# kaushik87599/Melo-GAN

Measured on AMD Instinct MI355X. Metric: piano-roll samples/sec (G+D step), batch=64 128x256 roll, higher is better.
Workload: dtype f32; 1 GPU; cfg2: 128x256 piano-roll, batch=64 per GPU, full G+D+emotion-D step (1 critic update incl. gradient penalty + 1 generator update); global_batch=64, T=256, C=128, parallelism=dp1, graph=True

## Files before the change

### include/melo_gan_hip.h

```cpp
#ifndef MELO_GAN_HIP_H
#define MELO_GAN_HIP_H

#include <stddef.h>
#include <stdint.h>

#ifdef __cplusplus
extern "C" {
#endif

typedef void* mg_stream_t;

enum { MG_ACT_NONE = 0, MG_ACT_RELU = 1, MG_ACT_LRELU = 2, MG_ACT_GELU = 3, MG_ACT_TANH = 4 };

typedef struct mg_epilogue {
    const float* bias;
    const float* scale;
    const float* shift;
    float* zout;
    int act;
    const float* gref;
    int gact;
    const float* emul;
    const float* gscale;
    int accumulate;
} mg_epilogue;

int mg_version(void);
const char* mg_last_error(void);

size_t mg_conv_workspace_bytes(int B, int Tout, int N);
int mg_conv1d_gather(const float* x, const float* w, float* y,
                     int B, int Tin, int Cin, int N, int K, int stride, int flip,
                     int w_sn, int w_sc, long xbs, long ybs,
                     const mg_epilogue* epi, void* work, size_t work_bytes, long lds_pad, mg_stream_t stream);

int mg_conv1d_scatter2(const float* x, const float* w, float* y,
                       int B, int Tin, int Cin, int N, int Tout,
                       int w_sn, int w_sc, long xbs, long ybs,
                       const mg_epilogue* epi, void* work, size_t work_bytes, mg_stream_t stream);

int mg_wq_relayout(const float* w, float* wq, int N, int Cc, int K, int w_sn, int w_sc, mg_stream_t stream);
int mg_conv16_supported(int B, int Tin, int Cin, int N, int transposed, int Tout);
int mg_conv16_plan(int B, int Tin, int N, int transposed, int* batch_rows_per_tile, int* part_rows, int* tile_rows);
int mg_conv16_poolable(int B, int Tin, int Cin, int N);
typedef struct mg_conv16_extra {
    float* part;
    float* pool;
    float pool_scale;
    int y_perm;
    const float* mix_real;
    const float* mix_alpha;
    float* mix_out;
    int mix_rows;
    const float* bnb_a;
    const float* bnb_z;
    const float* bnb_mean;
    const float* bnb_invstd;
    double* bnb_part;
    int bnb_act;
} mg_conv16_extra;
int mg_conv16(const float* x, const float* wq, float* y, int B, int Tin, int Cin, int N, int transposed, int Tout,
              long xbs, long ybs, const mg_epilogue* epi, const mg_conv16_extra* extra , mg_stream_t stream);
int mg_bn_train_bwd_parts(const double* part, int part_rows, const float* da, const float* a, const float* z, float* dz, long R,
                          int C, const float* gamma, const float* beta, const float* save_mean, const float* save_invstd,
                          float* dgamma, float* dbeta, int act, mg_stream_t stream);
int mg_bn_train_fwd_parts(const float* part, int part_rows_per_group, int groups, const float* z, float* a, long R, int C,
                          const float* gamma, const float* beta, float* running_mean, float* running_var, float momentum,
                          float eps, float* save_mean, float* save_invstd, int act, mg_stream_t stream);

#define MG_CHAIN_MAX_OPS 16
#define MG_CHAIN_SLOTS 6
#define MG_CHAIN_MAX_VEC 512
enum { MG_CH_LOAD = 1, MG_CH_STORE = 2, MG_CH_LAYERNORM = 3, MG_CH_LIN_FWD = 4, MG_CH_LIN_DGRAD = 5, MG_CH_SOFTMAX_CE = 6,
       MG_CH_DHEAD = 7, MG_CH_MEAN_T = 8, MG_CH_COPY = 9 };
typedef struct mg_chain_op {
    int kind;
    int a, b;
    int n0, n1;
    int act;
    int i0, i1;
    float f0;
    const float* p0; long ld0;
    const float* p1; long ld1;
    const float* p2; long ld2;
    const float* p3; long ld3;
    float* q0; long lq0;
    float* q1; long lq1;
    const int64_t* t0;
} mg_chain_op;
int mg_row_chain(const mg_chain_op* ops, int n_ops, int rows, mg_stream_t stream);
int mg_mean_scaled(const float* src, float* out, int n, float scale, mg_stream_t stream);
int mg_stamp(unsigned long long* dst, mg_stream_t stream);

size_t mg_linear_workspace_bytes(int M, int N, int K);
int mg_linear(const float* x, const float* w, float* y, int M, int K, int N, int w_sn, int w_sc,
              const mg_epilogue* epi, int perm_L, void* work, size_t work_bytes, mg_stream_t stream);
int mg_linear_route(int M, int K, int N, int w_sn, int w_sc, int perm_L, int x_aligned, int w_aligned,
                    int* kcontig, int* vec, int* ksplit);

int mg_conv1d_wino3_supported(int B, int T, int Cin, int N);
int mg_wino3_weights(const float* w, float* wt, int N, int Cin, long w_sn, long w_sc, int flip, mg_stream_t stream);
int mg_conv1d_wino3(const float* x, const float* wt, float* y, int B, int T, int Cin, int N, const mg_epilogue* epi,
                    long lds_pad, mg_stream_t stream);
#define MG_MAX_WINO_WJOBS 8
typedef struct mg_wino3_wjob {
    const float* w;
    float* wt;
    int N, Cin;
    long w_sn, w_sc;
    int flip;
} mg_wino3_wjob;
int mg_wino3_weights_multi(const mg_wino3_wjob* jobs, int n_jobs, mg_stream_t stream);

int mg_conv_tile_config(long m_rows, int N, int scatter2);
int mg_conv_plan(int B, int Tm, int Tout, int N, int Cin, int K, int stride, int scatter2, size_t work_bytes,
                 int* ksplit, int* cps);
int mg_conv_finish_vec(int N, long ybs, int tensors_aligned);

int mg_conv_thin_route(const float* x, long xbs, int Cin, int N, int K, int stride, int transposed);

typedef struct mg_epilogue_bf16 {
    const float* scale;
    const float* shift;
    void* zout;
    int act;
    const void* gref;
    int gact;
    const float* gscale;
    int accumulate;
} mg_epilogue_bf16;
int mg_wb_relayout(const float* w, void* wb, int N, int Cc, int K, int w_sn, int w_sc, int flip, mg_stream_t stream);
int mg_conv1d_s1_bf16_supported(int B, int T, int Cin, int N, int K);
int mg_conv1d_s1_bf16(const void* x, int x_f32, const void* wb, void* y, int y_f32, int B, int T, int Cin, int N, int K,
                      const mg_epilogue_bf16* epi, mg_stream_t stream);
int mg_meanT_fwd_bf16(const void* a, float* h, int B, int T, int C, mg_stream_t stream);
int mg_meanT_bwd_bf16(const float* dh, void* dz, const void* gref, int gact, const float* gscale, int B, int T, int C,
                      mg_stream_t stream);

size_t mg_wgrad_workspace_bytes(int A, int Bc, int K, int nb_total, int Ts);
int mg_wgrad(const float* s0, const float* l0, int nb0,
             const float* s1, const float* l1, int nb1,
             float* out, float* bias_out, int bias_from, int Ts, int Tl, int A, int Bc, int K, int stride,
             void* work, size_t work_bytes, mg_stream_t stream);

#define MG_MAX_WGRAD_JOBS 8
typedef struct mg_wgrad_job {
    const float* s0; const float* l0; int nb0;
    const float* s1; const float* l1; int nb1;
    float* out; float* bias_out; int bias_from;
    int Ts, Tl, A, Bc;
} mg_wgrad_job;
int mg_wgrad_multi(const mg_wgrad_job* jobs, int n_jobs, int K, int stride, void* work, size_t work_bytes,
                   mg_stream_t stream);

size_t mg_colsum_workspace_bytes(int C);
int mg_colsum(const float* x, long R, int C, float* sum, float* sumsq,
              void* work, size_t work_bytes, mg_stream_t stream);

size_t mg_bn_workspace_bytes(int C, int groups);
int mg_bn_train_fwd(const float* z, float* a, long R, int C, int groups, const float* gamma, const float* beta,
                    float* running_mean, float* running_var, float momentum, float eps,
                    float* save_mean, float* save_invstd, int act,
                    void* work, size_t work_bytes, mg_stream_t stream);
int mg_bn_train_bwd(const float* da, const float* a, const float* z, float* dz, long R, int C,
                    const float* gamma, const float* beta, const float* save_mean, const float* save_invstd,
                    float* dgamma, float* dbeta, int act,
                    void* work, size_t work_bytes, mg_stream_t stream);
int mg_bn_eval_fwd(const float* z, float* a, long R, int C, const float* gamma, const float* beta,
                   const float* running_mean, const float* running_var, float eps, int act,
                   mg_stream_t stream);
int mg_bn_fold(const float* gamma, const float* beta, const float* running_mean, const float* running_var,
               const float* conv_bias, float eps, float* scale, float* shift, int C, mg_stream_t stream);

int mg_meanT_fwd(const float* a, float* h, int B, int T, int C, mg_stream_t stream);
int mg_meanT_bwd(const float* dh, float* dz, int B, int T, int C, const float* gref, int gact, const float* gscale,
                 const float* mean_src, float* mean_out, int mean_n, float mean_scale, mg_stream_t stream);

int mg_layernorm_fwd(const float* x, float* y, float* xhat, int B, int D,
                     const float* gamma, const float* beta, float eps, mg_stream_t stream);
int mg_layernorm_bwd_params(const float* dy, const float* xhat, float* dgamma, float* dbeta,
                            int B, int D, mg_stream_t stream);

int mg_dhead_fwd(const float* f, const float* emb, const float* w, const float* bias, float* s,
                 int B, int Be, int F, int E, mg_stream_t stream);
int mg_dhead_bwd(const float* ds, const float* f, const float* w, float* dU, float* demb,
                 int B, int Be, int F, int E, int nb_emb, mg_stream_t stream);
// ... 238 lines not shown
```

### melo-gan_amd/_lib.py

```python
import ctypes as C
import os

_HERE = os.path.dirname(os.path.abspath(__file__))
LIB_PATH = os.path.join(_HERE, "libmelogan_hip.so")
if os.environ.get("MELO_LIB_VARIANT"):
    LIB_PATH = os.path.join(os.path.dirname(_HERE), "tools", "_build", "libmelogan_" + os.environ["MELO_LIB_VARIANT"] + ".so")

ACT_NONE, ACT_RELU, ACT_LRELU, ACT_GELU, ACT_TANH = 0, 1, 2, 3, 4

vp, i32, i64, f32, sz = C.c_void_p, C.c_int, C.c_long, C.c_float, C.c_size_t


class Epilogue(C.Structure):
    _fields_ = [("bias", vp), ("scale", vp), ("shift", vp), ("zout", vp), ("act", i32),
                ("gref", vp), ("gact", i32), ("emul", vp), ("gscale", vp), ("accumulate", i32)]


class EpilogueBf16(C.Structure):
    _fields_ = [("scale", vp), ("shift", vp), ("zout", vp), ("act", i32), ("gref", vp), ("gact", i32), ("gscale", vp),
                ("accumulate", i32)]


class Conv16Extra(C.Structure):
    _fields_ = [("part", vp), ("pool", vp), ("pool_scale", f32), ("y_perm", i32), ("mix_real", vp), ("mix_alpha", vp),
# ... 42 lines not shown


class WgradJob(C.Structure):
    _fields_ = [("s0", vp), ("l0", vp), ("nb0", i32), ("s1", vp), ("l1", vp), ("nb1", i32),
                ("out", vp), ("bias_out", vp), ("bias_from", i32), ("Ts", i32), ("Tl", i32), ("A", i32), ("Bc", i32)]


MAX_WGRAD_JOBS = 8


class WqEntry(C.Structure):
    _fields_ = [("start", i64), ("N", i32), ("Cc", i32), ("K", i32), ("w_sn", i32), ("w_sc", i32), ("dst", vp)]


MAX_WQ_ENTRIES = 8

MLP_MAX_HIDDEN, MLP_MAX_DIM, MLP_MAX_CLASSES = 4, 512, 32

VOICE_MAX_PARTIALS = 16


class Voice(C.Structure):
    _fields_ = [("n_partials", i32), ("mult", C.c_uint32 * VOICE_MAX_PARTIALS), ("weight", f32 * VOICE_MAX_PARTIALS),
                ("decay", f32 * VOICE_MAX_PARTIALS), ("attack", i32), ("release_tau", f32), ("release_len", i32), ("fs", f32)]


class MlpCls(C.Structure):
    _fields_ = [("n_hidden", i32), ("in_dim", i32), ("width", i32 * MLP_MAX_HIDDEN), ("n_classes", i32),
                ("w", vp * (MLP_MAX_HIDDEN + 1)), ("b", vp * (MLP_MAX_HIDDEN + 1)), ("z", vp * MLP_MAX_HIDDEN),
                ("a", vp * MLP_MAX_HIDDEN), ("dz", vp * MLP_MAX_HIDDEN), ("mask", vp * MLP_MAX_HIDDEN)]


SIGNATURES = {
    "mg_version": (i32, []),
    "mg_last_error": (C.c_char_p, []),
    "mg_conv_workspace_bytes": (sz, [i32, i32, i32]),
    "mg_conv1d_gather": (i32, [vp, vp, vp, i32, i32, i32, i32, i32, i32, i32, i32, i32, i64, i64, C.POINTER(Epilogue), vp, sz, i64, vp]),
    "mg_conv1d_scatter2": (i32, [vp, vp, vp, i32, i32, i32, i32, i32, i32, i32, i64, i64, C.POINTER(Epilogue), vp, sz, vp]),
    "mg_wq_relayout": (i32, [vp, vp, i32, i32, i32, i32, i32, vp]),
    "mg_conv16_supported": (i32, [i32, i32, i32, i32, i32, i32]),
    "mg_conv16_plan": (i32, [i32, i32, i32, i32, C.POINTER(i32), C.POINTER(i32), C.POINTER(i32)]),
    "mg_conv16": (i32, [vp, vp, vp, i32, i32, i32, i32, i32, i32, i64, i64, C.POINTER(Epilogue), C.POINTER(Conv16Extra), vp]),
    "mg_conv16_poolable": (i32, [i32, i32, i32, i32]),
    "mg_bn_train_fwd_parts": (i32, [vp, i32, i32, vp, vp, i64, i32, vp, vp, vp, vp, f32, f32, vp, vp, i32, vp]),
    "mg_linear_workspace_bytes": (sz, [i32, i32, i32]),
    "mg_linear": (i32, [vp, vp, vp, i32, i32, i32, i32, i32, C.POINTER(Epilogue), i32, vp, sz, vp]),
    "mg_conv_tile_config": (i32, [i64, i32, i32]),
    "mg_conv_plan": (i32, [i32, i32, i32, i32, i32, i32, i32, i32, sz, C.POINTER(i32), C.POINTER(i32)]),
    "mg_conv_finish_vec": (i32, [i32, i64, i32]),
    "mg_linear_route": (i32, [i32, i32, i32, i32, i32, i32, i32, i32, C.POINTER(i32), C.POINTER(i32), C.POINTER(i32)]),
    "mg_conv_thin_route": (i32, [vp, i64, i32, i32, i32, i32, i32]),
    "mg_wb_relayout": (i32, [vp, vp, i32, i32, i32, i32, i32, i32, vp]),
    "mg_conv1d_s1_bf16_supported": (i32, [i32, i32, i32, i32, i32]),
    "mg_conv1d_s1_bf16": (i32, [vp, i32, vp, vp, i32, i32, i32, i32, i32, i32, C.POINTER(EpilogueBf16), vp]),
    "mg_meanT_fwd_bf16": (i32, [vp, vp, i32, i32, i32, vp]),
    "mg_meanT_bwd_bf16": (i32, [vp, vp, vp, i32, vp, i32, i32, i32, vp]),
    "mg_wgrad_workspace_bytes": (sz, [i32, i32, i32, i32, i32]),
    "mg_wgrad": (i32, [vp, vp, i32, vp, vp, i32, vp, vp, i32, i32, i32, i32, i32, i32, i32, vp, sz, vp]),
    "mg_wgrad_multi": (i32, [vp, i32, i32, i32, vp, sz, vp]),
    "mg_colsum_workspace_bytes": (sz, [i32]),
    "mg_colsum": (i32, [vp, i64, i32, vp, vp, vp, sz, vp]),
    "mg_bn_workspace_bytes": (sz, [i32, i32]),
    "mg_bn_train_fwd": (i32, [vp, vp, i64, i32, i32, vp, vp, vp, vp, f32, f32, vp, vp, i32, vp, sz, vp]),
    "mg_bn_train_bwd": (i32, [vp, vp, vp, vp, i64, i32, vp, vp, vp, vp, vp, vp, i32, vp, sz, vp]),
    "mg_bn_train_bwd_parts": (i32, [vp, i32, vp, vp, vp, vp, i64, i32, vp, vp, vp, vp, vp, vp, i32, vp]),
    "mg_bn_eval_fwd": (i32, [vp, vp, i64, i32, vp, vp, vp, vp, f32, i32, vp]),
    "mg_bn_fold": (i32, [vp, vp, vp, vp, vp, f32, vp, vp, i32, vp]),
    "mg_meanT_fwd": (i32, [vp, vp, i32, i32, i32, vp]),
    "mg_layernorm_fwd": (i32, [vp, vp, vp, i32, i32, vp, vp, f32, vp]),
    "mg_layernorm_bwd_params": (i32, [vp, vp, vp, vp, i32, i32, vp]),
    "mg_dhead_fwd": (i32, [vp, vp, vp, vp, vp, i32, i32, i32, i32, vp]),
    "mg_dhead_bwd": (i32, [vp, vp, vp, vp, vp, i32, i32, i32, i32, i32, vp]),
    "mg_dhead_fwd_bwd": (i32, [vp, vp, vp, vp, vp, vp, vp, vp, i32, i32, i32, i32, i32, vp]),
    "mg_dhead_wgrad": (i32, [vp, vp, vp, vp, vp, vp, i32, i32, i32, i32, i32, vp, vp, f32, vp, vp, i32, vp]),
    "mg_meanT_bwd": (i32, [vp, vp, i32, i32, i32, vp, i32, vp, vp, vp, i32, f32, vp]),
    "mg_row_chain": (i32, [vp, i32, i32, vp]),
    "mg_mean_scaled": (i32, [vp, vp, i32, f32, vp]),
    "mg_stamp": (i32, [vp, vp]),
    "mg_spectral_norm_fwd": (i32, [vp, i32, i32, f32, vp]),
    "mg_spectral_norm_bwd": (i32, [vp, i32, vp]),
    "mg_conv1d_wino3_supported": (i32, [i32, i32, i32, i32]),
    "mg_wino3_weights": (i32, [vp, vp, i32, i32, i64, i64, i32, vp]),
    "mg_conv1d_wino3": (i32, [vp, vp, vp, i32, i32, i32, i32, vp, i64, vp]),
    "mg_wino3_weights_multi": (i32, [vp, i32, vp]),
    "mg_gp_interp": (i32, [vp, vp, vp, vp, i32, i64, vp]),
    "mg_gp_penalty": (i32, [vp, vp, vp, vp, f32, i32, i64, vp]),
    "mg_softmax_ce": (i32, [vp, vp, vp, vp, f32, i32, i32, vp]),
    "mg_axpby": (i32, [vp, vp, f32, f32, i64, vp]),
    "mg_copy_cols": (i32, [vp, i32, i32, vp, i32, i32, i32, i32, i32, vp]),
    "mg_transpose_bcl_blc": (i32, [vp, vp, i32, i32, i32, vp, i32, vp]),
    "mg_stage_rows": (i32, [vp, i32, i32, vp]),
    "mg_stage_rows_cursor": (i32, [vp, i32, i32, vp, i64, vp, vp, vp]),
    "mg_stage_augment": (i32, [vp, vp, i64, i32, i32, vp, vp, i32, vp, i64, vp, vp, vp, i32, C.POINTER(Augment), vp]),
    "mg_weighted_order": (i32, [vp, i64, vp, i64, C.c_uint64, C.c_uint64, vp]),
    "mg_ed_metrics_acc": (i32, [vp, vp, vp, i32, i32, vp, vp]),
    "mg_act_bwd": (i32, [vp, vp, i32, vp, vp, i64, vp]),
    "mg_rng_fill": (i32, [vp, i64, vp, i64, vp, i64, vp, i64, f32, C.c_uint64, vp, vp, vp, f32, f32, vp, i32, i32, vp, i64, vp, vp]),
    "mg_gen_inputs": (i32, [vp, vp, i32, vp, i32, vp, i32, vp, i32, f32, vp, i32, C.c_uint64, vp]),
    "mg_emotion_score": (i32, [vp, i32, i32, vp, vp, vp, vp, vp]),
    "mg_gen_inputs_mix": (i32, [vp, vp, vp, vp, i32, vp, i32, vp, i32, vp, i32, f32, vp, i32, C.c_uint64, vp]),
    "mg_path_d2": (i32, [vp, i32, i32, i32, vp, vp]),
    "mg_path_probs": (i32, [vp, vp, i32, i32, i32, i32, vp, vp, vp]),
    "mg_latent_rows": (i32, [vp, vp, i32, vp, i32, vp, vp, vp, vp, vp, vp, vp, vp, i32, i32, i32, C.c_uint64, vp, vp]),
    "mg_latent_cycle": (i32, [vp, vp, vp, i32, vp, i32, vp, vp, vp, i32, i32, vp, vp]),
    "mg_roll_encode": (i32, [vp, i64, vp, vp, i64, i32, i32, vp, vp, i64, vp, vp, vp]),
    "mg_window_votes": (i32, [vp, vp, i32, i32, i64, vp, vp, vp, vp, vp, vp]),
    "mg_ig_rows": (i32, [vp, vp, vp, vp, i32, i64, i32, i32, i32, i32, vp, vp, vp, vp]),
    "mg_ig_seed": (i32, [vp, vp, i64, i32, i32, i32, vp, vp, vp, vp, vp]),
    "mg_ig_accumulate": (i32, [vp, vp, i64, i32, i32, i32, vp, vp, vp, vp, vp, vp]),
    "mg_ig_rank": (i32, [vp, vp, i64, i32, vp, vp]),
    "mg_ig_rank_tile": (i32, []),
    "mg_motif_tokens": (i32, [vp, i64, i32, i32, vp, vp, vp]),
    "mg_motif_lcs": (i32, [vp, vp, i32, vp, vp, i64, i32, vp, vp, vp, vp, vp]),
    "mg_motif_rank": (i32, [vp, i32, i64, i32, vp, vp, vp]),
    "mg_motif_corpus_tile": (i32, []),
    "mg_render_notes": (i32, [vp, vp, vp, vp, vp, vp, vp, vp, i32, i64, C.POINTER(Voice), vp, vp, vp]),
    "mg_pcm_peak": (i32, [vp, vp, i32, i64, vp, vp]),
    "mg_pcm_quantise": (i32, [vp, vp, vp, i32, i64, f32, vp, vp]),
    "mg_eval_acc_words": (i64, [i32, i32]),
    "mg_eval_acc_workspace_bytes": (sz, [i32, i32, i32]),
    "mg_eval_acc_reset": (i32, [vp, i32, i32, vp]),
    "mg_eval_acc": (i32, [vp, vp, i32, i32, i32, vp, vp, vp, vp, vp, i32, vp, vp, sz, vp, vp]),
    "mg_eval_noise": (i32, [vp, i32, i32, vp, vp, i64, C.c_uint64, vp]),
    "mg_pair_workspace_bytes": (sz, [i64, i64, i32, i32]),
    "mg_pair_ksum": (i32, [vp, i64, vp, i64, i32, i32, vp, vp, sz, vp]),
    "mg_pair_knn": (i32, [vp, i64, vp, i64, i32, i32, i32, vp, vp, sz, vp]),
    "mg_pair_margin": (i32, [vp, i64, vp, i64, i32, vp, vp, vp, sz, vp]),
    "mg_scatter_rows_cursor": (i32, [vp, i32, i32, vp, i64, vp, vp, vp]),
    "mg_note_acc_words": (i64, [i32]),
    "mg_note_acc_reset": (i32, [vp, i32, vp]),
    "mg_note_stats": (i32, [vp, vp, i32, i32, i32, vp, i32, vp, vp, vp, i64, vp, vp, vp]),
    "mg_vae_eval_acc_words": (i64, [i32, i32]),
    "mg_vae_eval_acc_workspace_bytes": (sz, [i32, i32]),
    "mg_vae_eval_acc_reset": (i32, [vp, i32, i32, vp]),
    "mg_vae_eval_acc": (i32, [vp, vp, i32, i32, i32, vp, vp, i32, vp, i32, vp, vp, vp, i64, vp, vp, vp, sz, vp, vp]),
    "mg_cls_eval_acc_words": (i64, [i32, i32, i32]),
    "mg_cls_eval_acc_workspace_bytes": (sz, [i32, i32]),
    "mg_cls_eval_acc": (i32, [vp, vp, i32, i32, vp, i32, C.POINTER(C.c_double), i32, C.c_double, vp, vp, vp, vp, i64, vp, vp, vp, sz,
                              vp, vp]),
    "mg_cls_auroc_pairs": (i32, [vp, vp, i64, i32, vp, vp]),
    "mg_tsne_workspace_bytes": (sz, [i64]),
    "mg_tsne_affinities": (i32, [vp, i64, i32, f32, vp, vp, vp, sz, vp]),
    "mg_tsne_step": (i32, [vp, i64, vp, vp, vp, f32, f32, f32, vp, vp, vp, i64, vp, sz, vp]),
    "mg_adam_flat": (i32, [vp, vp, vp, vp, i64, f32, f32, f32, f32, f32, vp, f32, vp, i32, vp, vp, i32, vp]),
    "mg_ema_flat": (i32, [vp, vp, i64, C.c_double, i32, vp, C.c_double, vp]),
    "mg_mlp_cls_fwd_bwd": (i32, [C.POINTER(MlpCls), i32, vp, vp, vp, vp, i64, vp, i64, vp, i32, i32, i32, f32, C.c_uint64, vp, vp, f32, f32,
                                 vp, vp, vp, vp]),
    "mg_mlp_cls_wgrad_update": (i32, [C.POINTER(MlpCls), i32, vp, vp, C.POINTER(i64), C.POINTER(i64), i64, vp, vp, vp, vp, i32, f32, f32,
                                      f32, f32, f32, vp, vp, vp, vp, vp, vp, vp, vp]),
    "mg_grad_norm_workspace_bytes": (sz, [i64]),
    "mg_grad_norm_clip": (i32, [vp, i64, f32, vp, vp, sz, vp]),
    "mg_reparam_fwd": (i32, [vp, vp, vp, vp, i64, vp]),
    "mg_reparam_bwd": (i32, [vp, vp, vp, vp, vp, vp, vp, i64, vp]),
    "mg_vae_loss_workspace_bytes": (sz, []),
    "mg_vae_loss": (i32, [vp, vp, i64, vp, vp, i64, f32, vp, vp, vp, vp, vp, sz, vp]),
    "mg_graph_begin": (i32, [vp]),
    "mg_graph_end": (i32, [vp, C.POINTER(vp), i32]),
    "mg_graph_last_kernel_nodes": (i32, []),
    "mg_graph_launch": (i32, [vp, vp]),
    "mg_graph_destroy": (i32, [vp]),
    "mg_event_create": (i32, [C.POINTER(vp)]),
    "mg_event_record": (i32, [vp, vp]),
    "mg_event_elapsed_ms": (i32, [vp, vp, C.POINTER(f32)]),
    "mg_event_destroy": (i32, [vp]),
}

# ... 30 lines not shown
```

### melo-gan_amd/csrc/conv_wino.hip

```cpp
#include "common.h"
#include <type_traits>

namespace {

typedef unsigned u32x4 __attribute__((ext_vector_type(4)));

struct WinoP {
    const float* x;
    const float* wt;
    float* y;
    int B, T, Cin, N;
    int tiles_per_seq;
    int x_bytes, wt_bytes;
    mg_epilogue e;
};

constexpr int WP = 64;
constexpr int SX = 20;
constexpr int XT_FLOATS = 4 * WP * SX;
constexpr int WT_FLOATS = 4 * 4 * 64 * 4;
constexpr int BUF = XT_FLOATS + WT_FLOATS;

__global__ __launch_bounds__(256, 2) void wino3_kernel(const WinoP p) {
    extern __shared__ __attribute__((aligned(16))) float smem[];
    const int tid = threadIdx.x;
    const int lane = tid & 63;
    const int wave = __builtin_amdgcn_readfirstlane(tid >> 6);
    const int wm = wave >> 1, wn = wave & 1;
    const int b = blockIdx.x / p.tiles_per_seq;
    const int t0 = (blockIdx.x - b * p.tiles_per_seq) * (2 * WP);
    const int n0 = blockIdx.y * 64;

    auto lds4 = [&](int off) { return reinterpret_cast<f32x4*>(__builtin_assume_aligned(smem + off, 16)); };

    const int abase = (wm * 32 + (lane & 31)) * SX + 4 * (lane >> 5);
    const int bbase = XT_FLOATS + (lane >> 5) * 4 * 256 + (wn * 32 + (lane & 31)) * 4;

    f32x16 acc[4];
#pragma unroll
    for (int j = 0; j < 4; ++j)
#pragma unroll
        for (int r = 0; r < 16; ++r) acc[j][r] = 0.f;

    const __amdgpu_buffer_rsrc_t xrsrc = __builtin_amdgcn_make_buffer_rsrc(const_cast<float*>(p.x), 0, p.x_bytes, 0x00020000);
    const __amdgpu_buffer_rsrc_t wrsrc = __builtin_amdgcn_make_buffer_rsrc(const_cast<float*>(p.wt), 0, p.wt_bytes, 0x00020000);
    auto bload = [&](const __amdgpu_buffer_rsrc_t& rsrc, unsigned voff, unsigned soff) {
        const u32x4 v = __builtin_amdgcn_raw_buffer_load_b128(rsrc, voff, soff, 0);
        return f32x4{__uint_as_float(v[0]), __uint_as_float(v[1]), __uint_as_float(v[2]), __uint_as_float(v[3])};
    };

    const int pl = tid >> 2, q = tid & 3;
    unsigned xo[4];
#pragma unroll
    for (int i = 0; i < 4; ++i) {
        const int t = t0 - 1 + 2 * pl + i;
        xo[i] = (t >= 0 && t < p.T) ? ((unsigned)(b * p.T + t) * (unsigned)p.Cin + 4u * q) * 4u : 0x80000000u;
    }
    const int xl = pl * SX + 4 * q;
    unsigned wg[4];
    int wl[4];
#pragma unroll
    for (int i = 0; i < 4; ++i) {
        wg[i] = ((unsigned)(i * 4 + wave) * (unsigned)p.N * 4u + (unsigned)(n0 + lane) * 4u) * 4u;
        wl[i] = XT_FLOATS + (i * 4 + wave) * 256 + lane * 4;
    }
    f32x4 xr[4], ut[4], wr[4];
    auto x_soff = [&](int c0) { return 4u * (unsigned)c0; };
    auto w_soff = [&](int c0) { return (unsigned)c0 * (unsigned)p.N * 16u; };
    auto transform = [&]() {
        ut[0] = xr[0] - xr[2];
        ut[1] = xr[1] + xr[2];
        ut[2] = xr[2] - xr[1];
        ut[3] = xr[1] - xr[3];
    };
    auto store_x = [&](int j, int boff) { *lds4(boff + xl + j * WP * SX) = ut[j]; };
    auto store_w = [&](int i, int boff) { *lds4(boff + wl[i]) = wr[i]; };
    auto load_x = [&](int i, unsigned soff) { xr[i] = bload(xrsrc, xo[i], soff); };
    auto load_w = [&](int i, unsigned soff) { wr[i] = bload(wrsrc, wg[i], soff); };

    f32x4 fa[2], fb[2];
    auto frag_read = [&](int boff, int slot, f32x4& A, f32x4& Bv) {
        const int g = slot >> 2, j = slot & 3;
        A = *lds4(boff + abase + j * WP * SX + 8 * g);
        Bv = *lds4(boff + bbase + (8 * g + j) * 256);
    };

    const int c_last = p.Cin - 16;
    auto chunk = [&](auto parity, int c0) {
        constexpr int P = decltype(parity)::value;
        const int cur = P ? BUF : 0, oth = BUF - cur;
        const int cn = min(c0 + 32, c_last);
        const unsigned xs = x_soff(cn), ws = w_soff(cn);
#pragma unroll
        for (int m = 0; m < 32; ++m) {
            const int sl = m >> 2, s4 = m & 3, j = sl & 3;
            acc[j] = __builtin_amdgcn_mfma_f32_32x32x2f32(fa[sl & 1][s4], fb[sl & 1][s4], acc[j], 0, 0, 0);
            if (s4 == 0) {
                if (sl == 7) __syncthreads();
                if (sl + 1 < 8) frag_read(cur, sl + 1, fa[(sl + 1) & 1], fb[(sl + 1) & 1]);
                else frag_read(oth, 0, fa[0], fb[0]);
            } else {
                const int gap = sl * 3 + s4 - 1;
                if (gap == 0) transform();
                else if (gap <= 4) store_x(gap - 1, oth);
                else if (gap <= 12) {
                    if (gap & 1) load_x((gap - 5) >> 1, xs);
                    else store_w((gap - 6) >> 1, oth);
                } else if (gap <= 16) load_w(gap - 13, ws);
            }
            __builtin_amdgcn_sched_barrier(0);
        }
    };

#pragma unroll
    for (int i = 0; i < 4; ++i) load_x(i, x_soff(0));
#pragma unroll
    for (int i = 0; i < 4; ++i) load_w(i, w_soff(0));
    transform();
#pragma unroll
    for (int j = 0; j < 4; ++j) store_x(j, 0);
#pragma unroll
    for (int i = 0; i < 4; ++i) store_w(i, 0);
    {
        const int c1 = min(16, c_last);
#pragma unroll
        for (int i = 0; i < 4; ++i) load_x(i, x_soff(c1));
#pragma unroll
        for (int i = 0; i < 4; ++i) load_w(i, w_soff(c1));
    }
    __syncthreads();
    frag_read(0, 0, fa[0], fb[0]);
    for (int c0 = 0;;) {
        chunk(std::integral_constant<int, 0>{}, c0);
        c0 += 16;
        if (c0 >= p.Cin) break;
        chunk(std::integral_constant<int, 1>{}, c0);
        c0 += 16;
        if (c0 >= p.Cin) break;
    }

#pragma unroll
    for (int r = 0; r < 16; ++r) {
        const float m1 = acc[1][r], m2 = acc[2][r];
        acc[0][r] = acc[0][r] + m1 + m2;
        acc[3][r] = m1 - m2 - acc[3][r];
    }
    const mg_epilogue& E = p.e;
    const int n = n0 + wn * 32 + (lane & 31);
    const bool lin_tile = t0 + 2 * WP <= p.T;
    auto epilogue_pass = [&](auto lin_tag, auto ph_tag) {
        constexpr bool LIN = decltype(lin_tag)::value;
        constexpr int ph = decltype(ph_tag)::value;
        f32x16& a = acc[ph ? 3 : 0];
        const int ip0 = wm * 32 + 4 * (lane >> 5);
        const unsigned lin0 = (unsigned)((b * p.T + t0 + 2 * ip0 + ph) * p.N + n);
        auto index = [&](int r, unsigned& di) -> bool {
            const int dr = 2 * ((r & 3) + 8 * (r >> 2));
            di = lin0 + (unsigned)(dr * p.N);
            return LIN || (t0 + 2 * ip0 + ph + dr < p.T);
        };
        mg_epilogue_column<16>(E, a, n, index);
        unsigned di;
        if (E.accumulate) {
            float g[16];
#pragma unroll
            for (int r = 0; r < 16; ++r) g[r] = p.y[index(r, di) ? di : 0u];
#pragma unroll
            for (int r = 0; r < 16; ++r) a[r] += g[r];
        }
#pragma unroll
        for (int r = 0; r < 16; ++r)
            if (index(r, di)) p.y[di] = a[r];
    };
    if (lin_tile) {
        epilogue_pass(std::true_type{}, std::integral_constant<int, 0>{});
        epilogue_pass(std::true_type{}, std::integral_constant<int, 1>{});
    } else {
        epilogue_pass(std::false_type{}, std::integral_constant<int, 0>{});
        epilogue_pass(std::false_type{}, std::integral_constant<int, 1>{});
    }
}

__global__ void wino3_weights_kernel(const float* __restrict__ w, float* __restrict__ wt, int N, int Cin, long w_sn, long w_sc,
                                     int flip) {
    const long i = (long)blockIdx.x * blockDim.x + threadIdx.x;
    if (i >= (long)N * Cin) return;
    const int e = (int)(i & 3);
    const long r = i >> 2;
    const int n = (int)(r % N);
    const int cq = (int)(r / N);
    const float* g = w + (long)n * w_sn + (long)(4 * cq + e) * w_sc;
    const float g0 = g[flip ? 2 : 0], g1 = g[1], g2 = g[flip ? 0 : 2];
    const long o = ((long)cq * 4 * N + n) * 4 + e;
    const long ps = (long)N * 4;
    wt[o] = g0;
    wt[o + ps] = 0.5f * (g0 + g1 + g2);
    wt[o + 2 * ps] = 0.5f * (g0 - g1 + g2);
    wt[o + 3 * ps] = g2;
}

struct WinoWJobs { mg_wino3_wjob j[MG_MAX_WINO_WJOBS]; int n; };
__global__ void wino3_weights_multi_kernel(const WinoWJobs J) {
    const mg_wino3_wjob q = J.j[blockIdx.y];
    const long total = (long)q.N * q.Cin;
    for (long i = (long)blockIdx.x * blockDim.x + threadIdx.x; i < total; i += (long)gridDim.x * blockDim.x) {
        const int e = (int)(i & 3);
        const long r = i >> 2;
        const int n = (int)(r % q.N);
        const int cq = (int)(r / q.N);
        const float* g = q.w + (long)n * q.w_sn + (long)(4 * cq + e) * q.w_sc;
        const float g0 = g[q.flip ? 2 : 0], g1 = g[1], g2 = g[q.flip ? 0 : 2];
        const long o = ((long)cq * 4 * q.N + n) * 4 + e;
        const long ps = (long)q.N * 4;
        q.wt[o] = g0;
        q.wt[o + ps] = 0.5f * (g0 + g1 + g2);
        q.wt[o + 2 * ps] = 0.5f * (g0 - g1 + g2);
        q.wt[o + 3 * ps] = g2;
    }
}

}

extern "C" {

int mg_wino3_weights_multi(const mg_wino3_wjob* jobs, int n_jobs, mg_stream_t stream) {
    MG_CHECK_ARG(jobs && n_jobs > 0 && n_jobs <= MG_MAX_WINO_WJOBS, "mg_wino3_weights_multi: 1..%d jobs", MG_MAX_WINO_WJOBS);
    WinoWJobs J{};
    J.n = n_jobs;
    long mx = 0;
    for (int i = 0; i < n_jobs; ++i) {
        const mg_wino3_wjob& q = jobs[i];
        MG_CHECK_ARG(q.w && q.wt && q.N > 0 && q.Cin > 0 && (q.Cin & 3) == 0 && q.w_sn > 0 && q.w_sc > 0,
                     "mg_wino3_weights_multi: job %d: bad args (Cin must be a multiple of 4)", i);
        J.j[i] = q;
        const long t = (long)q.N * q.Cin;
        mx = t > mx ? t : mx;
    }
    long gx = mg_cdiv(mx, 256);
    gx = gx > 256 ? 256 : gx;
    hipLaunchKernelGGL(wino3_weights_multi_kernel, dim3((unsigned)gx, (unsigned)n_jobs), dim3(256), 0, (hipStream_t)stream, J);
    MG_CHECK_LAUNCH("wino3_weights_multi");
    return MG_OK;
}

int mg_conv1d_wino3_supported(int B, int T, int Cin, int N) {
    if (B <= 0 || T < 2 || (T & 1) || Cin < 16 || (Cin & 15) || N < 64 || (N & 63)) return 0;
    if ((long)B * T * Cin * 4 >= (1L << 31) || (long)B * T * N >= (1L << 31) || (long)Cin * N * 16 >= (1L << 31)) return 0;
    return 1;
}

int mg_wino3_weights(const float* w, float* wt, int N, int Cin, long w_sn, long w_sc, int flip, mg_stream_t stream) {
    MG_CHECK_ARG(w && wt && N > 0 && Cin > 0 && (Cin & 3) == 0, "mg_wino3_weights: bad args (Cin must be a multiple of 4)");
    const long total = (long)N * Cin;
    hipLaunchKernelGGL(wino3_weights_kernel, dim3((unsigned)mg_cdiv(total, 256)), dim3(256), 0, (hipStream_t)stream, w, wt, N,
                       Cin, w_sn, w_sc, flip);
    MG_CHECK_LAUNCH("wino3_weights");
    return MG_OK;
}

int mg_conv1d_wino3(const float* x, const float* wt, float* y, int B, int T, int Cin, int N, const mg_epilogue* epi,
                    long lds_pad, mg_stream_t stream) {
    MG_CHECK_ARG(x && wt && y, "mg_conv1d_wino3: null tensor");
    MG_CHECK_ARG(lds_pad >= 0 && lds_pad <= 120 * 1024, "mg_conv1d_wino3: lds_pad %ld outside 0..120 KiB", lds_pad);
    if (!mg_conv1d_wino3_supported(B, T, Cin, N)) {
        mg_set_error("mg_conv1d_wino3: unsupported shape B=%d T=%d Cin=%d N=%d (T even, Cin %% 16, N %% 64)", B, T, Cin, N);
        return MG_EUNSUP;
    }
    MG_CHECK_ARG(((((uintptr_t)x) | ((uintptr_t)wt)) & 15) == 0, "mg_conv1d_wino3: x / wt must be 16-byte aligned");
    WinoP p{};
    p.x = x; p.wt = wt; p.y = y;
    p.B = B; p.T = T; p.Cin = Cin; p.N = N;
    p.tiles_per_seq = (int)mg_cdiv(T, 2 * WP);
    p.x_bytes = (int)((long)B * T * Cin * 4);
    p.wt_bytes = (int)((long)Cin * N * 16);
    if (epi) {
        p.e = *epi;
        MG_CHECK_ARG(!(p.e.scale && !p.e.shift), "epilogue: scale without shift");
    }
    size_t lds = 2 * (size_t)BUF * sizeof(float);
    if (lds_pad > 0 && lds + (size_t)lds_pad <= 160 * 1024) lds += (size_t)lds_pad;
    static std::atomic<uint64_t> optin;
    if (int rc = mg_lds_optin(reinterpret_cast<const void*>(&wino3_kernel), optin)) return rc;
    dim3 grid((unsigned)(B * p.tiles_per_seq), (unsigned)(N / 64));
    hipLaunchKernelGGL(wino3_kernel, grid, dim3(256), lds, (hipStream_t)stream, p);
    MG_CHECK_LAUNCH("wino3");
    return MG_OK;
}

}
```

### melo-gan_amd/ops.py

```python
from __future__ import annotations

import ctypes as C
import functools
import math
from typing import Optional

import torch

from . import _lib as L
from ._lib import ACT_NONE, ACT_RELU, ACT_LRELU, ACT_GELU, ACT_TANH, Epilogue

Tensor = torch.Tensor


def _stream() -> C.c_void_p:
    return C.c_void_p(torch.cuda.current_stream().cuda_stream)


def _p(t: Optional[Tensor]):
    return None if t is None else C.c_void_p(t.data_ptr())


def _chk(t: Tensor, name: str, shape=None, dtype=torch.float32):
    if not isinstance(t, torch.Tensor) or not t.is_cuda:
# ... 80 lines not shown
        raise ValueError(f"y: expected (B={B}, >={Tout}, {N}), got {tuple(y.shape)}")
    need = (N - 1) * w_sn + (Cin - 1) * w_sc + K
    if w.numel() < need:
        raise ValueError(f"w: numel {w.numel()} < {need} implied by strides")
    e = epilogue((B, Tout, N), N, **epi)
    if y.shape[1] != Tout and (e.zout or e.gref or e.emul):
        raise ValueError("padded y cannot be combined with elementwise epilogue tensors")
    lib = L.load()
    def sym():
        thin = lib.mg_conv_thin_route(_p(x), Tin * Cin, Cin, N, K, stride, 0)
        if thin:
            return _THIN_SYMBOLS[thin] % "false"
        return "conv_wgemm_kernel<%d,%d,false,%s,%s>" % (
            stride, K, "true" if w_sc < w_sn else "false",
            {22: "2,2", 12: "1,2", 11: "1,1"}[lib.mg_conv_tile_config(B * Tout, N, 0)])
    work = _conv_work(lib, B, Tout, N, Cin, x.device)
    def launch():
        return lib.mg_conv1d_gather(_p(x), _p(w), _p(y), B, Tin, Cin, N, K, stride, 1 if flip else 0, w_sn, w_sc,
                                    Tin * Cin, y.shape[1] * N, C.byref(e), _p(work),
                                    work.numel() if work is not None else 0, lds_pad, _stream())
    with _observe(sym, 2.0 * B * Tout * N * Cin * K, launch):
        rc = launch()
    L.check(rc, "mg_conv1d_gather")
    return y


def conv_plan(B: int, Tin: int, Cin: int, N: int, K: int, stride: int, scatter2: bool = False, odd: bool = False):
    Tout = (2 * Tin - (1 if odd else 0)) if scatter2 else (Tin + 2 * ((K - 1) // 2) - K) // stride + 1
    ks, cps = C.c_int(), C.c_int()
    L.check(L.load().mg_conv_plan(B, Tin if scatter2 else Tout, Tout, N, Cin, K, stride, 1 if scatter2 else 0,
                                  conv_work_bytes(B, Tout, N, Cin), C.byref(ks), C.byref(cps)), "mg_conv_plan")
    return ks.value, cps.value


def conv_finish_vec(y: Tensor, N: int, *tensors) -> bool:
    work = workspace(1, y.device, "conv")
    aligned = all(t is None or t.data_ptr() % 16 == 0 for t in (work, y) + tensors)
    return bool(L.load().mg_conv_finish_vec(N, y.shape[1] * N, int(aligned)))


def wino3_supported(B: int, T: int, Cin: int, N: int) -> bool:
    return bool(L.load().mg_conv1d_wino3_supported(B, T, Cin, N))


def wino3_weights(w: Tensor, N: int, Cin: int, w_sn: int, w_sc: int, flip: bool = False, out: Optional[Tensor] = None) -> Tensor:
    _chk(w, "w")
    if w.numel() < (N - 1) * w_sn + (Cin - 1) * w_sc + 3:
        raise ValueError("wino3_weights: w smaller than its strides imply")
    wt = out if out is not None else torch.empty(Cin // 4, 4, N, 4, device=w.device, dtype=torch.float32)
    _chk(wt, "wt", (Cin // 4, 4, N, 4))
    L.check(L.load().mg_wino3_weights(_p(w), _p(wt), N, Cin, w_sn, w_sc, 1 if flip else 0, _stream()), "mg_wino3_weights")
    return wt


def wino3_weights_multi(jobs):
    if not 0 < len(jobs) <= L.MAX_WINO_WJOBS:
        raise ValueError(f"wino3_weights_multi: 1..{L.MAX_WINO_WJOBS} jobs")
    arr = (L.WinoWJob * len(jobs))()
    for a, (w, wt, N, Cin, w_sn, w_sc, flip) in zip(arr, jobs):
        _chk(w, "w")
        _chk(wt, "wt", (Cin // 4, 4, N, 4))
        if w.numel() < (N - 1) * w_sn + (Cin - 1) * w_sc + 3:
            raise ValueError("wino3_weights_multi: w smaller than its strides imply")
        a.w, a.wt, a.N, a.Cin, a.w_sn, a.w_sc, a.flip = w.data_ptr(), wt.data_ptr(), N, Cin, w_sn, w_sc, 1 if flip else 0
    L.check(L.load().mg_wino3_weights_multi(arr, len(jobs), _stream()), "mg_wino3_weights_multi")


def conv_wino3(x: Tensor, wt: Tensor, y: Tensor, lds_pad: int = 0, **epi) -> Tensor:
    _chk(x, "x")
    _chk(wt, "wt")
    _chk(y, "y")
    B, T, Cin = x.shape
    N = wt.shape[2]
    if tuple(wt.shape) != (Cin // 4, 4, N, 4) or tuple(y.shape) != (B, T, N):
        raise ValueError(f"conv_wino3: wt {tuple(wt.shape)} / y {tuple(y.shape)} do not fit x {tuple(x.shape)}")
    e = epilogue((B, T, N), N, **epi)
    lib = L.load()
    def launch():
        return lib.mg_conv1d_wino3(_p(x), _p(wt), _p(y), B, T, Cin, N, C.byref(e), lds_pad, _stream())
    with _observe(lambda: "wino3_kernel", 2.0 * B * T * N * Cin * 3, launch):
        rc = launch()
    L.check(rc, "mg_conv1d_wino3")
    return y


def conv_scatter2(x: Tensor, w: Tensor, y: Tensor, N: int, w_sn: int, w_sc: int, odd: bool = False, **epi) -> Tensor:
    _chk(x, "x")
    _chk(w, "w")
    _chk(y, "y")
    B, Tin, Cin = x.shape
    Tout = 2 * Tin - (1 if odd else 0)
    if y.dim() != 3 or y.shape[0] != B or y.shape[2] != N or y.shape[1] < Tout:
        raise ValueError(f"y: expected (B={B}, >={Tout}, {N}), got {tuple(y.shape)}")
    need = (N - 1) * w_sn + (Cin - 1) * w_sc + 5
    if w.numel() < need:
        raise ValueError(f"w: numel {w.numel()} < {need} implied by strides")
    e = epilogue((B, Tout, N), N, **epi)
    if y.shape[1] != Tout and (e.zout or e.gref or e.emul):
        raise ValueError("padded y cannot be combined with elementwise epilogue tensors")
    lib = L.load()
    def sym():
        thin = lib.mg_conv_thin_route(_p(x), Tin * Cin, Cin, N, 5, 2, 1)
        if thin:
            return _THIN_SYMBOLS[thin] % "true"
        return "conv_wgemm_kernel<2,5,true,%s,%s>" % (
            "true" if w_sc < w_sn else "false", "1,2" if lib.mg_conv_tile_config(B * Tin, N, 1) == 12 else "1,1")
    work = _conv_work(lib, B, Tout, N, Cin, x.device)
    with _observe(sym, 2.0 * B * Tin * N * Cin * 5):
        rc = lib.mg_conv1d_scatter2(_p(x), _p(w), _p(y), B, Tin, Cin, N, Tout, w_sn, w_sc, Tin * Cin, y.shape[1] * N,
                                    C.byref(e), _p(work), work.numel() if work is not None else 0, _stream())
    L.check(rc, "mg_conv1d_scatter2")
    return y


def conv1d_fwd(x, w, y, stride, **epi):
    Cout, Cin, K = w.shape
    if x.shape[2] != Cin:
        raise ValueError("conv1d_fwd: channel mismatch")
    return conv_gather(x, w, y, Cout, K, stride, Cin * K, K, **epi)


def conv1d_dgrad(dy, w, dx, stride, lds_pad: int = 0, **epi):
    Cout, Cin, K = w.shape
    if dy.shape[2] != Cout:
        raise ValueError("conv1d_dgrad: channel mismatch")
    if stride == 1:
        return conv_gather(dy, w, dx, Cin, K, 1, K, Cin * K, flip=True, lds_pad=lds_pad, **epi)
    if K != 5 or lds_pad:
        raise ValueError("stride-2 dgrad needs K=5 and takes no lds_pad")
    odd = dx.shape[1] == 2 * dy.shape[1] - 1
    return conv_scatter2(dy, w, dx, Cin, K, Cin * K, odd=odd, **epi)


def convT1d_fwd(x, w, y, **epi):
    Cin, Cout, K = w.shape
    if x.shape[2] != Cin or K != 5:
        raise ValueError("convT1d_fwd: shape mismatch")
    return conv_scatter2(x, w, y, Cout, K, Cout * K, **epi)


def convT1d_dgrad(dy, w, dx, **epi):
    Cin, Cout, K = w.shape
    if dy.shape[2] != Cout:
        raise ValueError("convT1d_dgrad: channel mismatch")
    return conv_gather(dy, w, dx, Cin, K, 2, Cout * K, K, **epi)


def wq_relayout(w: Tensor, wq: Tensor, N: int, Cc: int, K: int, w_sn: int, w_sc: int) -> Tensor:
    _chk(w, "w")
    _chk(wq, "wq")
    if wq.numel() != N * Cc * K or w.numel() < (N - 1) * w_sn + (Cc - 1) * w_sc + K or Cc % 4:
        raise ValueError("wq_relayout: size mismatch")
    L.check(L.load().mg_wq_relayout(_p(w), _p(wq), N, Cc, K, w_sn, w_sc, _stream()), "mg_wq_relayout")
    return wq


def conv16_supported(B: int, Tin: int, Cin: int, N: int, transposed: bool, Tout: int = 0) -> bool:
    return bool(L.load().mg_conv16_supported(B, Tin, Cin, N, 1 if transposed else 0, Tout))


def conv16_poolable(B: int, Tin: int, Cin: int, N: int) -> bool:
    return bool(L.load().mg_conv16_poolable(B, Tin, Cin, N))


def conv16_pool(x: Tensor, wq: Tensor, y: Tensor, N: int, pool: Tensor, scale: float, **epi) -> Tensor:
    return conv16(x, wq, y, N, False, pool=(pool, scale), **epi)
# ... 2242 lines not shown
```

Measured before the change: 81330 samples/s.

## Make Winograd conv kernel persistent with cross-tile prefetch of next tile's inputs

Turns the wino3 conv into a persistent kernel: the grid is capped at the occupancy-derived slot count and each workgroup loops over tiles with a stride of G. The input and weight prefetch runs into the next tile's first channel chunk, so the load pipeline is not drained between tiles. The kernel is templated on whether Cin/16 is even, with a runtime-offset chunk path for the odd case. It also adds a planning API and optional timestamp instrumentation. The aim is to cut tail effects and per-tile pipeline warm-up, at the cost of some extra register pressure and control overhead.

```diff
diff --git a/include/melo_gan_hip.h b/include/melo_gan_hip.h
--- a/include/melo_gan_hip.h
+++ b/include/melo_gan_hip.h
@@ -102,6 +102,7 @@
 int mg_wino3_weights(const float* w, float* wt, int N, int Cin, long w_sn, long w_sc, int flip, mg_stream_t stream);
 int mg_conv1d_wino3(const float* x, const float* wt, float* y, int B, int T, int Cin, int N, const mg_epilogue* epi,
                     long lds_pad, mg_stream_t stream);
+int mg_conv1d_wino3_plan(int B, int T, int Cin, int N, long lds_pad, int* workgroups, int* tiles);
 #define MG_MAX_WINO_WJOBS 8
 typedef struct mg_wino3_wjob {
     const float* w;
diff --git a/melo-gan_amd/_lib.py b/melo-gan_amd/_lib.py
--- a/melo-gan_amd/_lib.py
+++ b/melo-gan_amd/_lib.py
@@ -148,6 +148,7 @@
     "mg_conv1d_wino3_supported": (i32, [i32, i32, i32, i32]),
     "mg_wino3_weights": (i32, [vp, vp, i32, i32, i64, i64, i32, vp]),
     "mg_conv1d_wino3": (i32, [vp, vp, vp, i32, i32, i32, i32, vp, i64, vp]),
+    "mg_conv1d_wino3_plan": (i32, [i32, i32, i32, i32, i64, vp, vp]),
     "mg_wino3_weights_multi": (i32, [vp, i32, vp]),
     "mg_gp_interp": (i32, [vp, vp, vp, vp, i32, i64, vp]),
     "mg_gp_penalty": (i32, [vp, vp, vp, vp, f32, i32, i64, vp]),
diff --git a/melo-gan_amd/csrc/conv_wino.hip b/melo-gan_amd/csrc/conv_wino.hip
--- a/melo-gan_amd/csrc/conv_wino.hip
+++ b/melo-gan_amd/csrc/conv_wino.hip
@@ -1,9 +1,21 @@
 #include "common.h"
+#include <mutex>
 #include <type_traits>
+#include <vector>
 
 namespace {
 
 typedef unsigned u32x4 __attribute__((ext_vector_type(4)));
+
+#ifdef MG_STAMPS
+__device__ long long* mg_wino_stamp_buf = nullptr;
+#define MG_STAMP(k)                                                                                    \
+    do {                                                                                               \
+        if (threadIdx.x == 0 && mg_wino_stamp_buf) mg_wino_stamp_buf[(long)blockIdx.x * 16 + (k)] = wall_clock64(); \
+    } while (0)
+#else
+#define MG_STAMP(k)
+#endif
 
 struct WinoP {
     const float* x;
@@ -11,6 +23,9 @@
     float* y;
     int B, T, Cin, N;
     int tiles_per_seq;
+    int m_tiles;
+    int total;
+    int G;
     int x_bytes, wt_bytes;
     mg_epilogue e;
 };
@@ -21,17 +36,23 @@
 constexpr int WT_FLOATS = 4 * 4 * 64 * 4;
 constexpr int BUF = XT_FLOATS + WT_FLOATS;
 
+template <bool EVEN>
 __global__ __launch_bounds__(256, 2) void wino3_kernel(const WinoP p) {
     extern __shared__ __attribute__((aligned(16))) float smem[];
     const int tid = threadIdx.x;
+    MG_STAMP(0);
     const int lane = tid & 63;
     const int wave = __builtin_amdgcn_readfirstlane(tid >> 6);
     const int wm = wave >> 1, wn = wave & 1;
-    const int b = blockIdx.x / p.tiles_per_seq;
-    const int t0 = (blockIdx.x - b * p.tiles_per_seq) * (2 * WP);
-    const int n0 = blockIdx.y * 64;
-
-    auto lds4 = [&](int off) { return reinterpret_cast<f32x4*>(__builtin_assume_aligned(smem + off, 16)); };
+    int tile = blockIdx.x, b, t0, n0;
+    auto tile_coords = [&](int L, int& bb, int& tt, int& nn) {
+        const int nt = L / p.m_tiles, m = L - nt * p.m_tiles;
+        bb = m / p.tiles_per_seq;
+        tt = (m - bb * p.tiles_per_seq) * (2 * WP);
+        nn = nt * 64;
+    };
+    tile_coords(tile, b, t0, n0);
+
 
     const int abase = (wm * 32 + (lane & 31)) * SX + 4 * (lane >> 5);
     const int bbase = XT_FLOATS + (lane >> 5) * 4 * 256 + (wn * 32 + (lane & 31)) * 4;
@@ -41,6 +62,7 @@
     for (int j = 0; j < 4; ++j)
 #pragma unroll
         for (int r = 0; r < 16; ++r) acc[j][r] = 0.f;
+    asm volatile("" : "+v"(acc[0]), "+v"(acc[1]), "+v"(acc[2]), "+v"(acc[3]));
 
     const __amdgpu_buffer_rsrc_t xrsrc = __builtin_amdgcn_make_buffer_rsrc(const_cast<float*>(p.x), 0, p.x_bytes, 0x00020000);
     const __amdgpu_buffer_rsrc_t wrsrc = __builtin_amdgcn_make_buffer_rsrc(const_cast<float*>(p.wt), 0, p.wt_bytes, 0x00020000);
@@ -51,19 +73,29 @@
 
     const int pl = tid >> 2, q = tid & 3;
     unsigned xo[4];
-#pragma unroll
-    for (int i = 0; i < 4; ++i) {
-        const int t = t0 - 1 + 2 * pl + i;
-        xo[i] = (t >= 0 && t < p.T) ? ((unsigned)(b * p.T + t) * (unsigned)p.Cin + 4u * q) * 4u : 0x80000000u;
-    }
     const int xl = pl * SX + 4 * q;
     unsigned wg[4];
-    int wl[4];
-#pragma unroll
-    for (int i = 0; i < 4; ++i) {
-        wg[i] = ((unsigned)(i * 4 + wave) * (unsigned)p.N * 4u + (unsigned)(n0 + lane) * 4u) * 4u;
-        wl[i] = XT_FLOATS + (i * 4 + wave) * 256 + lane * 4;
-    }
+    const int wl = XT_FLOATS + wave * 256 + lane * 4;
+    auto load_addrs = [&](int bb, int tt, int nn) {
+#pragma unroll
+        for (int i = 0; i < 4; ++i) {
+            const int t = tt - 1 + 2 * pl + i;
+            xo[i] = (t >= 0 && t < p.T) ? ((unsigned)(bb * p.T + t) * (unsigned)p.Cin + 4u * q) * 4u : 0x80000000u;
+            wg[i] = ((unsigned)(i * 4 + wave) * (unsigned)p.N * 4u + (unsigned)(nn + lane) * 4u) * 4u;
+        }
+    };
+    load_addrs(b, t0, n0);
+    int lt = tile, lc = 0;
+    auto advance = [&]() {
+        if (lc + 16 < p.Cin) lc += 16;
+        else if (lt + p.G < p.total) {
+            lt += p.G;
+            lc = 0;
+            int bb, tt, nn;
+            tile_coords(lt, bb, tt, nn);
+            load_addrs(bb, tt, nn);
+        }
+    };
     f32x4 xr[4], ut[4], wr[4];
     auto x_soff = [&](int c0) { return 4u * (unsigned)c0; };
     auto w_soff = [&](int c0) { return (unsigned)c0 * (unsigned)p.N * 16u; };
@@ -73,44 +105,53 @@
         ut[2] = xr[2] - xr[1];
         ut[3] = xr[1] - xr[3];
     };
-    auto store_x = [&](int j, int boff) { *lds4(boff + xl + j * WP * SX) = ut[j]; };
-    auto store_w = [&](int i, int boff) { *lds4(boff + wl[i]) = wr[i]; };
+    auto ldsb = [&](int byte) { return reinterpret_cast<f32x4*>(__builtin_assume_aligned(reinterpret_cast<char*>(smem) + byte, 16)); };
+    auto store_x = [&](int j, int xb) { *ldsb(xb + 4 * j * WP * SX) = ut[j]; };
+    auto store_w = [&](int i, int wb) { *ldsb(wb + 4 * i * 4 * 256) = wr[i]; };
     auto load_x = [&](int i, unsigned soff) { xr[i] = bload(xrsrc, xo[i], soff); };
     auto load_w = [&](int i, unsigned soff) { wr[i] = bload(wrsrc, wg[i], soff); };
 
     f32x4 fa[2], fb[2];
-    auto frag_read = [&](int boff, int slot, f32x4& A, f32x4& Bv) {
+    auto frag_read = [&](int ab, int bb, int slot, f32x4& A, f32x4& Bv) {
         const int g = slot >> 2, j = slot & 3;
-        A = *lds4(boff + abase + j * WP * SX + 8 * g);
-        Bv = *lds4(boff + bbase + (8 * g + j) * 256);
-    };
-
-    const int c_last = p.Cin - 16;
-    auto chunk = [&](auto parity, int c0) {
-        constexpr int P = decltype(parity)::value;
-        const int cur = P ? BUF : 0, oth = BUF - cur;
-        const int cn = min(c0 + 32, c_last);
-        const unsigned xs = x_soff(cn), ws = w_soff(cn);
+        A = *ldsb(ab + 4 * (j * WP * SX + 8 * g));
+        Bv = *ldsb(bb + 4 * (8 * g + j) * 256);
+    };
+
+    auto chunk_body = [&](const int a_cur, const int b_cur, const int a_oth, const int b_oth, const int x_oth, const int w_oth,
+                          const unsigned xs, const unsigned ws) {
 #pragma unroll
         for (int m = 0; m < 32; ++m) {
             const int sl = m >> 2, s4 = m & 3, j = sl & 3;
             acc[j] = __builtin_amdgcn_mfma_f32_32x32x2f32(fa[sl & 1][s4], fb[sl & 1][s4], acc[j], 0, 0, 0);
             if (s4 == 0) {
                 if (sl == 7) __syncthreads();
-                if (sl + 1 < 8) frag_read(cur, sl + 1, fa[(sl + 1) & 1], fb[(sl + 1) & 1]);
-                else frag_read(oth, 0, fa[0], fb[0]);
+                if (sl + 1 < 8) frag_read(a_cur, b_cur, sl + 1, fa[(sl + 1) & 1], fb[(sl + 1) & 1]);
+                else frag_read(a_oth, b_oth, 0, fa[0], fb[0]);
             } else {
                 const int gap = sl * 3 + s4 - 1;
                 if (gap == 0) transform();
-                else if (gap <= 4) store_x(gap - 1, oth);
+                else if (gap <= 4) store_x(gap - 1, x_oth);
                 else if (gap <= 12) {
                     if (gap & 1) load_x((gap - 5) >> 1, xs);
-                    else store_w((gap - 6) >> 1, oth);
+                    else store_w((gap - 6) >> 1, w_oth);
                 } else if (gap <= 16) load_w(gap - 13, ws);
             }
             __builtin_amdgcn_sched_barrier(0);
         }
     };
+    auto chunk = [&](auto parity, const unsigned xs, const unsigned ws) {
+        constexpr int cur = decltype(parity)::value ? BUF : 0, oth = BUF - cur;
+        chunk_body(4 * (cur + abase), 4 * (cur + bbase), 4 * (oth + abase), 4 * (oth + bbase), 4 * (oth + xl), 4 * (oth + wl), xs, ws);
+    };
+    auto chunk_rt = [&](const int cur, const unsigned xs, const unsigned ws) {
+        const int oth = BUF - cur;
+        int a_cur = 4 * (cur + abase), b_cur = 4 * (cur + bbase), a_oth = 4 * (oth + abase), b_oth = 4 * (oth + bbase),
+            x_oth = 4 * (oth + xl), w_oth = 4 * (oth + wl);
+        asm volatile("" : "+v"(a_cur), "+v"(b_cur), "+v"(a_oth), "+v"(b_oth), "+v"(x_oth), "+v"(w_oth));
+        __builtin_amdgcn_sched_barrier(0);
+        chunk_body(a_cur, b_cur, a_oth, b_oth, x_oth, w_oth, xs, ws);
+    };
 
 #pragma unroll
     for (int i = 0; i < 4; ++i) load_x(i, x_soff(0));
@@ -118,26 +159,44 @@
     for (int i = 0; i < 4; ++i) load_w(i, w_soff(0));
     transform();
 #pragma unroll
-    for (int j = 0; j < 4; ++j) store_x(j, 0);
-#pragma unroll
-    for (int i = 0; i < 4; ++i) store_w(i, 0);
-    {
-        const int c1 = min(16, c_last);
-#pragma unroll
-        for (int i = 0; i < 4; ++i) load_x(i, x_soff(c1));
-#pragma unroll
-        for (int i = 0; i < 4; ++i) load_w(i, w_soff(c1));
-    }
+    for (int j = 0; j < 4; ++j) store_x(j, 4 * xl);
+#pragma unroll
+    for (int i = 0; i < 4; ++i) store_w(i, 4 * wl);
+    advance();
+#pragma unroll
+    for (int i = 0; i < 4; ++i) load_x(i, x_soff(lc));
+#pragma unroll
+    for (int i = 0; i < 4; ++i) load_w(i, w_soff(lc));
     __syncthreads();
-    frag_read(0, 0, fa[0], fb[0]);
-    for (int c0 = 0;;) {
-        chunk(std::integral_constant<int, 0>{}, c0);
-        c0 += 16;
-        if (c0 >= p.Cin) break;
-        chunk(std::integral_constant<int, 1>{}, c0);
-        c0 += 16;
-        if (c0 >= p.Cin) break;
-    }
+    MG_STAMP(2);
+#ifdef MG_STAMPS
+    const long long clk2 = clock64();
+#endif
+    frag_read(4 * abase, 4 * bbase, 0, fa[0], fb[0]);
+    const mg_epilogue& E = p.e;
+    int cur = 0;
+    for (;;) {
+    if constexpr (EVEN) {
+        for (int c0 = 0; c0 < p.Cin; c0 += 32) {
+            advance();
+            chunk(std::integral_constant<int, 0>{}, x_soff(lc), w_soff(lc));
+            advance();
+            chunk(std::integral_constant<int, 1>{}, x_soff(lc), w_soff(lc));
+        }
+    } else {
+        for (int c0 = 0; c0 < p.Cin; c0 += 16) {
+            advance();
+            chunk_rt(cur, x_soff(lc), w_soff(lc));
+            cur = BUF - cur;
+        }
+    }
+#ifdef MG_STAMPS
+    if (tile == (int)blockIdx.x) {
+        MG_STAMP(3);
+        if (threadIdx.x == 0 && mg_wino_stamp_buf) mg_wino_stamp_buf[(long)blockIdx.x * 16 + 14] = clock64() - clk2;
+    }
+    else if (tile == (int)blockIdx.x + p.G) MG_STAMP(6);
+#endif
 
 #pragma unroll
     for (int r = 0; r < 16; ++r) {
@@ -145,7 +204,6 @@
         acc[0][r] = acc[0][r] + m1 + m2;
         acc[3][r] = m1 - m2 - acc[3][r];
     }
-    const mg_epilogue& E = p.e;
     const int n = n0 + wn * 32 + (lane & 31);
     const bool lin_tile = t0 + 2 * WP <= p.T;
     auto epilogue_pass = [&](auto lin_tag, auto ph_tag) {
@@ -179,6 +237,18 @@
         epilogue_pass(std::false_type{}, std::integral_constant<int, 0>{});
         epilogue_pass(std::false_type{}, std::integral_constant<int, 1>{});
     }
+#ifdef MG_STAMPS
+    if (tile == (int)blockIdx.x) MG_STAMP(5);
+#endif
+    tile += p.G;
+    if (tile >= p.total) break;
+    tile_coords(tile, b, t0, n0);
+#pragma unroll
+    for (int j = 0; j < 4; ++j)
+#pragma unroll
+        for (int r = 0; r < 16; ++r) acc[j][r] = 0.f;
+    }
+    MG_STAMP(4);
 }
 
 __global__ void wino3_weights_kernel(const float* __restrict__ w, float* __restrict__ wt, int N, int Cin, long w_sn, long w_sc,
@@ -219,6 +289,42 @@
     }
 }
 
+size_t wino_lds_bytes(long lds_pad) {
+    size_t lds = 2 * (size_t)BUF * sizeof(float);
+    if (lds_pad > 0 && lds + (size_t)lds_pad <= 160 * 1024) lds += (size_t)lds_pad;
+    return lds;
+}
+
+template <bool EVEN>
+int wino_slots(size_t lds, int* slots) {
+    static std::atomic<uint64_t> optin;
+    if (int rc = mg_lds_optin(reinterpret_cast<const void*>(&wino3_kernel<EVEN>), optin)) return rc;
+    struct Entry { size_t lds; int slots; };
+    struct Dev { std::mutex m; std::vector<Entry> e; };
+    static Dev devs[64];
+    int dev = 0;
+    MG_HIP(hipGetDevice(&dev));
+    Dev* d = dev >= 0 && dev < 64 ? &devs[dev] : nullptr;
+    if (d) {
+        std::lock_guard<std::mutex> g(d->m);
+        for (const Entry& e : d->e)
+            if (e.lds == lds) { *slots = e.slots; return MG_OK; }
+    }
+    int cus = 0, per_cu = 0;
+    MG_HIP(hipDeviceGetAttribute(&cus, hipDeviceAttributeMultiprocessorCount, dev));
+    MG_HIP(hipOccupancyMaxActiveBlocksPerMultiprocessor(&per_cu, wino3_kernel<EVEN>, 256, lds));
+    const int s = (cus > 0 ? cus : 1) * (per_cu > 0 ? per_cu : 1);
+    if (d) {
+        std::lock_guard<std::mutex> g(d->m);
+        d->e.push_back({lds, s});
+    }
+    *slots = s;
+    return MG_OK;
+}
+int wino_slots(int Cin, size_t lds, int* slots) {
+    return (Cin & 16) == 0 ? wino_slots<true>(lds, slots) : wino_slots<false>(lds, slots);
+}
+
 }
 
 extern "C" {
@@ -271,20 +377,42 @@
     p.x = x; p.wt = wt; p.y = y;
     p.B = B; p.T = T; p.Cin = Cin; p.N = N;
     p.tiles_per_seq = (int)mg_cdiv(T, 2 * WP);
+    p.m_tiles = B * p.tiles_per_seq;
+    p.total = p.m_tiles * (N / 64);
     p.x_bytes = (int)((long)B * T * Cin * 4);
     p.wt_bytes = (int)((long)Cin * N * 16);
     if (epi) {
         p.e = *epi;
         MG_CHECK_ARG(!(p.e.scale && !p.e.shift), "epilogue: scale without shift");
     }
-    size_t lds = 2 * (size_t)BUF * sizeof(float);
-    if (lds_pad > 0 && lds + (size_t)lds_pad <= 160 * 1024) lds += (size_t)lds_pad;
-    static std::atomic<uint64_t> optin;
-    if (int rc = mg_lds_optin(reinterpret_cast<const void*>(&wino3_kernel), optin)) return rc;
-    dim3 grid((unsigned)(B * p.tiles_per_seq), (unsigned)(N / 64));
-    hipLaunchKernelGGL(wino3_kernel, grid, dim3(256), lds, (hipStream_t)stream, p);
+    const size_t lds = wino_lds_bytes(lds_pad);
+    int slots = 0;
+    if (int rc = wino_slots(Cin, lds, &slots)) return rc;
+    p.G = p.total < slots ? p.total : slots;
+    if ((Cin & 16) == 0) hipLaunchKernelGGL(wino3_kernel<true>, dim3((unsigned)p.G), dim3(256), lds, (hipStream_t)stream, p);
+    else hipLaunchKernelGGL(wino3_kernel<false>, dim3((unsigned)p.G), dim3(256), lds, (hipStream_t)stream, p);
     MG_CHECK_LAUNCH("wino3");
     return MG_OK;
 }
 
-}
+#ifdef MG_STAMPS
+int mg_dbg_set_wino_stamps(long long* buf) {
+    return hipMemcpyToSymbol(HIP_SYMBOL(mg_wino_stamp_buf), &buf, sizeof(buf)) == hipSuccess ? 0 : 1;
+}
+#endif
+
+int mg_conv1d_wino3_plan(int B, int T, int Cin, int N, long lds_pad, int* workgroups, int* tiles) {
+    MG_CHECK_ARG(lds_pad >= 0 && lds_pad <= 120 * 1024, "mg_conv1d_wino3_plan: lds_pad %ld outside 0..120 KiB", lds_pad);
+    if (!mg_conv1d_wino3_supported(B, T, Cin, N)) {
+        mg_set_error("mg_conv1d_wino3_plan: unsupported shape B=%d T=%d Cin=%d N=%d (T even, Cin %% 16, N %% 64)", B, T, Cin, N);
+        return MG_EUNSUP;
+    }
+    int slots = 0;
+    if (int rc = wino_slots(Cin, wino_lds_bytes(lds_pad), &slots)) return rc;
+    const int total = B * (int)mg_cdiv(T, 2 * WP) * (N / 64);
+    if (workgroups) *workgroups = total < slots ? total : slots;
+    if (tiles) *tiles = total;
+    return MG_OK;
+}
+
+}
diff --git a/melo-gan_amd/ops.py b/melo-gan_amd/ops.py
--- a/melo-gan_amd/ops.py
+++ b/melo-gan_amd/ops.py
@@ -186,6 +186,12 @@
         rc = launch()
     L.check(rc, "mg_conv1d_wino3")
     return y
+
+
+def wino3_plan(B: int, T: int, Cin: int, N: int, lds_pad: int = 0):
+    wg, tiles = C.c_int(), C.c_int()
+    L.check(L.load().mg_conv1d_wino3_plan(B, T, Cin, N, lds_pad, C.byref(wg), C.byref(tiles)), "mg_conv1d_wino3_plan")
+    return wg.value, tiles.value
 
 
 def conv_scatter2(x: Tensor, w: Tensor, y: Tensor, N: int, w_sn: int, w_sc: int, odd: bool = False, **epi) -> Tensor:
```

After: 80600 samples/s. About the same (-0.9%).
